# LulinZhang/BRDF-NeRF

Measured on AMD Instinct MI355X. Metric: train rays/sec (+ MFMA% of roofline), spsbrdf-nerf 64 samples/ray, 1/2/4/8 MI355X, higher is better.
Workload: dtype bf16; 1 GPU; BASELINE config 2: Djibouti-shaped synthetic rays, spsbrdf-nerf lambert train step (pass1 64 + guided 64 samples/ray, F=512, 8 Siren layers, PE10, ds_lambda=10), 4096 rays/GPU/step (4096 rays per global step, weak scaling); rays_per_gpu=4096, n_samples=64, guided_samples=64, parallelism=dp1, settle_steps=218

## Files before the change

brdf_nerf_amd/csrc/diag.h:

```cpp
#ifdef BN_SWITCH
BN_SWITCH(BN_PHASE_TIMING)
BN_SWITCH(BN_PHASE_TIMING_WGRAD)
BN_SWITCH(BN_CLOCK_STAMP)
BN_SWITCH(BN_CLOCK_STAMP_WGRAD)
BN_SWITCH(BN_TIMELINE)
BN_SWITCH(BN_GEMM_PRIO)
BN_SWITCH(BN_NO_NT_STASH)
BN_SWITCH(BN_NO_PINGPONG)
BN_SWITCH(BN_BWD_NO_PINGPONG)
BN_SWITCH(BN_FWD_DEPTH_TRAIN)
BN_SWITCH(BN_BWD_DEPTH)
BN_SWITCH(BN_BWD_PP_DEPTH)
BN_SWITCH(BN_BWD_D_AT)
BN_SWITCH(BN_NO_FLAT_COMPOSITE)
BN_SWITCH(SKINNY_SPLITS)
BN_SWITCH(BN_W2_BLOCKS)
BN_SWITCH(BN_DIAG_D8_IN_F32)
BN_SWITCH(BN_PROBE_NO_A)
BN_SWITCH(BN_PROBE_NO_B)
BN_SWITCH(BN_PROBE_NO_D)
BN_SWITCH(BN_PROBE_NO_RIDE)
BN_SWITCH(BN_ABLATION_BUILD)
#else
#ifndef BN_GEMM_PRIO
#define BN_GEMM_PRIO 1
#endif
#ifndef BN_FWD_DEPTH_TRAIN
#define BN_FWD_DEPTH_TRAIN 6
#endif
#ifndef BN_BWD_DEPTH
#define BN_BWD_DEPTH 2
#endif
#ifndef BN_BWD_PP_DEPTH
#define BN_BWD_PP_DEPTH 6
#endif
#ifndef BN_BWD_D_AT
#define BN_BWD_D_AT 0
#endif
#ifndef SKINNY_SPLITS
#define SKINNY_SPLITS 256
#endif
#ifndef BN_W2_BLOCKS
#define BN_W2_BLOCKS 256
#endif
#endif
```

brdf_nerf_amd/csrc/field_bwd.hip:

```cpp
#include "field_kernels.h"
#include "field_wgrad.h"

int bn_field_adjoint_backward(const bn_field_desc *desc, const bn_field_params *params, const void *packed, const bn_points *pts,
                              const float *d_out, void *stash, void *stream);

__device__ unsigned int g_bwd_fault;
unsigned int bn_bwd_fault_read(hipStream_t) {
  unsigned int v = 0u;
  if (hipMemcpyFromSymbol(&v, HIP_SYMBOL(g_bwd_fault), sizeof(unsigned int), 0, hipMemcpyDeviceToHost) != hipSuccess) return 0x80000000u;
  return v;
}
const unsigned int *bn_bwd_fault_ptr() {
  void *p = nullptr;
  return hipGetSymbolAddress(&p, HIP_SYMBOL(g_bwd_fault)) == hipSuccess ? (const unsigned int *)p : nullptr;
}

BN_PH_DEFINE_READER(bn_debug_phase_read_bwd)
BN_CLK_DEFINE(bn_debug_clock_read_bwd)

struct BwdArgs {
  FieldGeom g;
  bn_field_desc d;
  bn_field_params p;
  PackedLayout pl;
// ... 127 lines not shown
  const int N = g.pass_N[p];
  const int pc0 = wave * 32 * NTW;
  if (pc0 >= N) return;
  const int hl = pc0 / g.H2, hd = 2 * p + hl;
  const int nout = A.d.head_out[hd];
  const float *w2 = A.p.head_w2[hd];
  const char *DGs = A.stash + A.sl.DG[p] + (size_t)tile * dtile_bytes<DK>(BM, F);
#pragma unroll
  for (int nt = 0; nt < NTW; ++nt) {
    f32x4 wa[2][3], wb[2][3];
#pragma unroll
    for (int gp = 0; gp < 2; ++gp) {
      const int nl = pc0 + nt * 32 + 16 * gp + 4 * h - hl * g.H2;
#pragma unroll
      for (int c = 0; c < 3; ++c) {
        wa[gp][c] = c < nout ? *(const f32x4 *)(w2 + (size_t)c * g.H2 + nl) : f32x4{0, 0, 0, 0};
        wb[gp][c] = c < nout ? *(const f32x4 *)(w2 + (size_t)c * g.H2 + nl + 8) : f32x4{0, 0, 0, 0};
      }
    }
#pragma unroll
    for (int mt = 0; mt < MT; ++mt) {
      const int m = mt * 32 + r;
      const float d0 = DPH[m * BN_DPH + hd * 3 + 0], d1 = DPH[m * BN_DPH + hd * 3 + 1], d2 = DPH[m * BN_DPH + hd * 3 + 2];
      const DPiece<DK> pc = dpiece_load<DK>(DGs + dpiece_off<DK, MT, NTW>(wave, nt, mt, lane));
#pragma unroll
      for (int gp = 0; gp < 2; ++gp) {
        const int n0 = pc0 + nt * 32 + 16 * gp + 4 * h;
        float dg[8];
        dpiece_get<DK>(pc, gp, g.act, 1.f, dg);
        float va[4], vb[4];
#pragma unroll
        for (int e = 0; e < 4; ++e) {
          va[e] = (d0 * wa[gp][0][e] + d1 * wa[gp][1][e] + d2 * wa[gp][2][e]) * dg[e];
          vb[e] = (d0 * wb[gp][0][e] + d1 * wb[gp][1][e] + d2 * wb[gp][2][e]) * dg[4 + e];
        }
        *(vec4 *)(ACT + (size_t)m * LDA + n0) = to_vec4(T(), va[0], va[1], va[2], va[3]);
        *(vec4 *)(ACT + (size_t)m * LDA + n0 + 8) = to_vec4(T(), vb[0], vb[1], vb[2], vb[3]);
      }
    }
  }
}

template <typename T, int MT, int NT, int WAVES, bool D16>
__global__ __launch_bounds__(WAVES * 64, 2) void field_bwd_kernel(const BwdArgs A) {
  typedef typename DKind<T, D16>::type DK;
  typedef typename Elem<T>::vec4 vec4;
  constexpr int BM = MT * 32;
  extern __shared__ __attribute__((aligned(16))) char smem[];
  const FieldGeom &g = A.g;
  const int F = g.F, LDA = F + Elem<T>::kPad, KSF = F / 16;
  T *ACT = (T *)smem;
  float *DPH = (float *)(ACT + (size_t)BM * LDA);
  float *DPT = DPH + BM * BN_DPH;
  int *WR = (int *)(DPT + BM * 4), *RD = WR + 2;

  const int tid = threadIdx.x, lane = tid & 63, wave = tid >> 6, r = lane & 31, h = lane >> 5;
  const int64_t tile = blockIdx.x, m0 = tile * BM, M = A.M;
  const T *packed = (const T *)A.packed;
  constexpr int DP = (NT == 2 && WAVES == 8 && Elem<T>::kFastMath) ? (BN_BWD_PP_DEPTH | BN_GEMM_AFFINE) : BwdDepth<T>::value;
  constexpr int NPRE = std::is_same<DK, DK8>::value ? NT : 1;
  BN_PH_DECL
  BN_CLK_BEGIN

  const float gs = chain_scale(A.amax);
  if (tid < 16) WR[tid] = 0;
  if (tid < BM) {
    const int m = tid;
    const int64_t gm = m0 + m;
    float dph[BN_DPH], dpt[4];
    bwd_dpre(A, gm, dph, dpt);
    float *sh = (float *)(A.stash + A.sl.dpre_head) + gm * BN_DPH;
    float *st = (float *)(A.stash + A.sl.dpre_trunk) + gm * 4;
#pragma unroll
    for (int i = 0; i < BN_DPH; ++i) { DPH[m * BN_DPH + i] = dph[i] * gs; sh[i] = dph[i]; }
#pragma unroll
    for (int i = 0; i < 4; ++i) { DPT[m * 4 + i] = dpt[i] * gs; st[i] = dpt[i]; }
  }
  __syncthreads();
  BN_PH(0)

  const int ncol0 = wave * 32 * NT;
  const bool wave_on = ncol0 < F;
  const int n_on = F / (32 * NT) < WAVES ? F / (32 * NT) : WAVES;
  const bool ride = NT == 2 ? true : tile_copy_exact(F, n_on, WAVES);
  f32x16 acc[NT][MT];
  zero_acc<MT, NT>(acc);
  const float zr = (A.an && A.amax) ? gs / grad_scale_from(A.amax + 1, BN_GS_TARGET_ADJ) : 1.f;

  for (int p = 0; p < g.n_pass; ++p) {
    if (g.pass_heads[p] == 2) bwd_head_dG<T, MT, NT, D16>(A, p, ACT, DPH, m0, tile);
    else bwd_head_dG<T, MT, BN_SINGLE_HEAD_NTW(NT), D16>(A, p, ACT, DPH, m0, tile);
    BN_PH(1)
    __syncthreads();
    BN_PH(2)
    BN_PH(3)
    const int KSp = g.pass_N[p] / 16;
    tile_to_global<T>(ACT, LDA, (T *)(A.stash + A.sl.dG[p]) + (size_t)m0 * g.pass_N[p], g.pass_N[p], BM, g.pass_N[p]);
    if (wave_on) gemm_seg<T, MT, NT, DP>(acc, packed + A.pl.bwd_head[p] + (size_t)(ncol0 / 32) * KSp * 512, KSp, ACT, LDA, lane);
    BN_PH(4)
    __syncthreads();
    BN_PH(5)
  }
  if (wave_on && !g.fold) {
#pragma unroll
    for (int nt = 0; nt < NT; ++nt)
#pragma unroll
      for (int gq = 0; gq < 4; ++gq) {
        const int n = ncol0 + nt * 32 + 8 * gq + 4 * h;
#pragma unroll
        for (int mt = 0; mt < MT; ++mt) {
          const int m = mt * 32 + r;
          *(vec4 *)(ACT + (size_t)m * LDA + n) =
              to_vec4(T(), acc[nt][mt][4 * gq], acc[nt][mt][4 * gq + 1], acc[nt][mt][4 * gq + 2], acc[nt][mt][4 * gq + 3]);
        }
      }
  }
  BN_PH(6)
  __syncthreads();
// ... 83 lines not shown
            }
#pragma unroll
            for (int e = 0; e < 8; ++e) v[e] += zb[e] * zr;
          }
          if constexpr (NATZ) {
            const typename Elem<T>::frag q = cvt8(T(), v);
            *(vec4 *)(ACT + (size_t)m * LDA + n0) = __builtin_shufflevector(q, q, 0, 1, 2, 3);
            *(vec4 *)(ACT + (size_t)m * LDA + n0 + 8) = __builtin_shufflevector(q, q, 4, 5, 6, 7);
            stash_store_buf(Zr, voff, ((((wave_u * NT + nt) * MT + mt) * 2 + gp) * 1024), q);
          } else {
            *(vec4 *)(ACT + (size_t)m * LDA + n0) = to_vec4(T(), v[0], v[1], v[2], v[3]);
            *(vec4 *)(ACT + (size_t)m * LDA + n0 + 8) = to_vec4(T(), v[4], v[5], v[6], v[7]);
          }
        }
      }
  };
  {
    if (!g.fold) {
      zero_acc<MT, NT>(acc);
      T *fdst = (T *)(A.stash + A.sl.dfeats) + (size_t)m0 * F;
      if (!ride) tile_to_global<T>(ACT, LDA, fdst, F, BM, F);
      if (wave_on) {
        load_D(g.L - 1, 0, NPRE);
        const size_t off = A.pl.bwd_feats + (size_t)(ncol0 / 32) * KSF * 512;
        if (ride) {
          TileCopyExact<T> zcopy(ACT, LDA, fdst, F, F, tid, WAVES * 64);
          gemm_seg<T, MT, NT, DP>(acc, packed + off, KSF, ACT, LDA, lane, zcopy);
        } else {
          gemm_seg<T, MT, NT, DP>(acc, packed + off, KSF, ACT, LDA, lane);
        }
        load_D(g.L - 1, NPRE, NT);
      }
    } else if (wave_on) {
      load_D(g.L - 1, 0, NT);
    }
    BN_PH(9)
    __syncthreads();
    BN_PH(10)
    if (wave_on) epilogue(g.L - 1, std::true_type());
    BN_PH(11)
    __syncthreads();
    BN_PH(12)
  }
  for (int l = g.L - 1; l >= 1; --l) {
    const int it = g.L - 1 - l;
    const int lo = l - 1;
    zero_acc<MT, NT>(acc);
    T *zdst = (T *)(A.stash + A.sl.dZ[l]) + (size_t)m0 * F;
    if (!NATZ && !ride) tile_to_global<T>(ACT, LDA, zdst, F, BM, F);
    if (wave_on) {
      if (!PING || BN_BWD_D_AT == 0) load_D(lo, 0, NPRE);
      const size_t off = A.pl.bwd_trunk[l] + (size_t)(ncol0 / 32) * KSF * 512;
      if constexpr (PING) {
        pp_wait(WR + 0, 4 * it, &g_bwd_fault);
        if (grp == 1) pp_wait(RD + 0, 4 * (it + 1), &g_bwd_fault);
        BN_PH(12)
        __builtin_amdgcn_s_setprio(1);
        if constexpr (sizeof(T) == 2) {
          gemm_fixed<T, MT, NT, (DP & (BN_GEMM_AFFINE - 1)), 32, 16>(acc, packed + off, KSF, 0, ACT, LDA, lane, [&]() {
            pp_signal(RD + 0 + grp, lane);
            pp_wait(WR + 1, 4 * it, &g_bwd_fault);
            if (BN_BWD_D_AT == 1) load_D(lo, 0, NPRE);
          });
        }
        __builtin_amdgcn_s_setprio(0);
        pp_signal(RD + 2 + grp, lane);
        if (BN_BWD_D_AT == 2) load_D(lo, 0, NPRE);
      } else if (!NATZ && ride) {
        TileCopyExact<T> zcopy(ACT, LDA, zdst, F, F, tid, WAVES * 64);
        gemm_seg<T, MT, NT, DP>(acc, packed + off, KSF, ACT, LDA, lane, zcopy);
      } else {
        gemm_seg<T, MT, NT, DP>(acc, packed + off, KSF, ACT, LDA, lane);
      }
      load_D(lo, NPRE, NT);
    }
    BN_PH(9)
    if constexpr (PING) {
      pp_wait(RD + 2 * grp + 0, 4 * (it + 1), &g_bwd_fault);
      pp_wait(RD + 2 * grp + 1, 4 * (it + 1), &g_bwd_fault);
    } else {
      __syncthreads();
    }
    BN_PH(10)
    if (wave_on) epilogue(lo, std::false_type());
    BN_PH(11)
    if constexpr (PING) pp_signal(WR + grp, lane);
    else __syncthreads();
    BN_PH(12)
  }
  if (PING) __syncthreads();
  if (!NATZ) tile_to_global<T>(ACT, LDA, (T *)(A.stash + A.sl.dZ[0]) + (size_t)m0 * F, F, BM, F);
  BN_PH(13)
#ifndef BN_PHASE_TIMING_WGRAD
  BN_PH_FLUSH
#endif
#ifndef BN_CLOCK_STAMP_WGRAD
  BN_CLK_END
#endif
}

template <typename T, int MT, int NT, int WAVES, bool D16> static int launch_bwd_k(const BwdArgs &a, int64_t tiles, hipStream_t st) {
  constexpr int BM = MT * 32;
  const size_t lds = (size_t)BM * (a.g.F + Elem<T>::kPad) * sizeof(T) + (size_t)BM * (BN_DPH + 4) * sizeof(float) + 64;
  if (int e = bn_configure_lds((const void *)field_bwd_kernel<T, MT, NT, WAVES, D16>, lds, "field_bwd")) return e;
  BnProfScope prof_(BN_K_BWD_CHAIN, st);
  field_bwd_kernel<T, MT, NT, WAVES, D16><<<dim3((unsigned)tiles), WAVES * 64, lds, st>>>(a);
  BN_LAUNCH_CHECK("field_bwd");
  return 0;
}
template <typename T, int MT, int NT, int WAVES> static int launch_bwd(const BwdArgs &a, int64_t tiles, hipStream_t st) {
  if constexpr (std::is_same<T, f16>::value) {
    if (a.g.dsz == 2) return launch_bwd_k<T, MT, NT, WAVES, true>(a, tiles, st);
  }
  return launch_bwd_k<T, MT, NT, WAVES, false>(a, tiles, st);
}

extern "C" int bn_field_backward(const bn_field_desc *desc, const bn_field_params *params, const void *packed,
                                 const bn_points *pts, const float *out, const float *d_out, void *stash,
                                 const bn_field_grads *G, void *stream) {
  return bn_field_backward_parts(desc, params, packed, pts, out, d_out, stash, G, BN_BWD_ALL, stream);
}

extern "C" int bn_field_backward_parts(const bn_field_desc *desc, const bn_field_params *params, const void *packed,
                                       const bn_points *pts, const float *out, const float *d_out, void *stash,
                                       const bn_field_grads *G, int32_t parts, void *stream) {
  BwdArgs a;
  if (int e = bn_make_geom(desc, &a.g)) return e;
  if (const int f = bn_field_fault_seen()) {
    bn_set_error("field_backward: an earlier %s launch lost an LDS hand-over (pp_wait timed out): its results are invalid",
                 (f & 1) ? "forward" : "backward");
    return BN_ELAUNCH;
  }
  a.an = desc->normal_an ? 1 : 0;
  BN_REQUIRE(pts && pts->n_points > 0 && packed && out && d_out && stash && G, "field_backward: null argument");
  BN_REQUIRE(parts > 0 && (parts & ~BN_BWD_ALL) == 0, "field_backward: parts=%d", parts);
  BN_REQUIRE(pts->point_offset == 0 && (pts->total_points == 0 || pts->total_points == pts->n_points),
             "field_backward: the backward runs over a whole point set (point_offset = 0)");
  BN_REQUIRE(pts->seg1_points == 0 || (pts->rays && pts->z && pts->z2 && pts->n_samples2 > 0 && pts->seg1_points < pts->n_points &&
                                       pts->seg1_points % pts->n_samples == 0 && (pts->n_points - pts->seg1_points) % pts->n_samples2 == 0),
// ... 165 lines not shown
```

brdf_nerf_amd/csrc/field_fwd.hip:

```cpp
#include "field_kernels.h"

struct FwdArgs {
  FieldGeom g;
  bn_field_desc d;
  bn_field_params p;
  PackedLayout pl;
  StashLayout sl;
  const void *packed;
  bn_points pts;
  float *out;
  char *stash;
  int sigma_only;
};

#define BN_INV_2PI 0.15915494309189535f

__device__ unsigned int g_fwd_fault;
static unsigned int *g_fault_host = nullptr;
static unsigned int g_fwd_launches = 0;
const unsigned int *bn_fwd_fault_ptr() {
  void *p = nullptr;
  return hipGetSymbolAddress(&p, HIP_SYMBOL(g_fwd_fault)) == hipSuccess ? (const unsigned int *)p : nullptr;
}

// ... 190 lines not shown
  constexpr int BM = MT * 32;
  constexpr int PADE = Elem<T>::kPad;
  constexpr bool FAST = Elem<T>::kFastMath;
  constexpr bool NATY = Elem<T>::kNativeY;
  constexpr int DP = FwdDepth<T, KEEP>::value;
  extern __shared__ __attribute__((aligned(16))) char smem[];
  const FieldGeom &g = A.g;
  const int F = g.F, LDA = F + PADE, KP = g.KP, LDP = KP + PADE;
  T *ACT = (T *)smem;
  T *PE = ACT + (size_t)BM * LDA;
  float *RED = (float *)(PE + (size_t)BM * LDP);

  const int tid = threadIdx.x, lane = tid & 63, wave = tid >> 6;
  const int r = lane & 31, h = lane >> 5;
  const int64_t tile = blockIdx.x, m0 = tile * BM, M = A.pts.n_points;
  const T *packed = (const T *)A.packed;
  constexpr bool keep = KEEP;
  BN_PH_DECL
  BN_CLK_BEGIN

  {
    constexpr int NP = (WAVES * 64) / BM;
    const int m = tid % BM, part = tid / BM;
    const int64_t gm = m0 + m;
    float x[3] = {0.f, 0.f, 0.f};
    if (gm < M) {
      if (A.pts.xyz) {
        x[0] = A.pts.xyz[gm * 3 + 0]; x[1] = A.pts.xyz[gm * 3 + 1]; x[2] = A.pts.xyz[gm * 3 + 2];
      } else {
        const int64_t ray = gm / A.pts.n_samples;
        const float *rr = A.pts.rays + ray * A.pts.ray_stride;
        const float zz = A.pts.z[gm];
        x[0] = rr[0] + rr[3] * zz; x[1] = rr[1] + rr[4] * zz; x[2] = rr[2] + rr[5] * zz;
      }
    }
    T *row = PE + (size_t)m * LDP;
    if (g.pe_freqs > 0) {
      for (int k = part; k < g.pe_freqs; k += NP) {
        const float f = (float)(1 << k);
#pragma unroll
        for (int c = 0; c < 3; ++c) {
          float s, co;
          sincos_t<FAST>(f * x[c], s, co);
          row[6 * k + c] = (T)s;
          row[6 * k + 3 + c] = (T)co;
        }
      }
      if (part == 0)
        for (int k = g.P; k < KP; ++k) row[k] = (T)0.f;
    } else if (part == 0) {
      for (int k = 0; k < KP; ++k) row[k] = (T)(k < 3 ? x[k] : 0.f);
    }
  }
  if (tid < 8) ((int *)RED)[tid] = 0;
  __syncthreads();
  if (keep) tile_to_global<T>(PE, LDP, (T *)(A.stash + A.sl.pe) + (size_t)m0 * KP, KP, BM, KP);
  BN_PH(0)

  const int ncol0 = wave * 32 * NT;
  const bool wave_on = ncol0 < F;
  const int KSP = KP / 16, KSF = F / 16;
  f32x16 acc[NT][MT];

  const int n_on = F / (32 * NT) < WAVES ? F / (32 * NT) : WAVES;
  const bool ride = NT == 2 ? true : tile_copy_exact(F, n_on, WAVES);
#ifndef BN_NO_PINGPONG
  constexpr bool PING = NT == 2 && WAVES == 8 && FAST;
#else
  constexpr bool PING = false;
#endif
  int *WR = (int *)RED, *RD = WR + 2;
  const int grp = wave >> 2;
  BN_TL_DECL((char *)RED + 64 + 4096)
  float *BIASL = (float *)((char *)RED + 64) + wave * 128;
  float bnext = 0.f;
  const int wave_u = __builtin_amdgcn_readfirstlane(wave);
  if constexpr (PING) BIASL[lane] = A.p.trunk_b[0][ncol0 + lane] * act_prescale<FAST>(g.act, 30.f);
  for (int l = 0; l < g.L; ++l) {
    BN_TL(0)
    if constexpr (PING) {
      if (l + 1 < g.L) bnext = A.p.trunk_b[l + 1][ncol0 + lane];
      const float *bl = BIASL + (l & 1) * 64 + 4 * h;
#pragma unroll
      for (int nt = 0; nt < NT; ++nt)
#pragma unroll
        for (int gp = 0; gp < 2; ++gp) {
          const f32x4 b0 = *(const f32x4 *)(bl + nt * 32 + 16 * gp), b1 = *(const f32x4 *)(bl + nt * 32 + 16 * gp + 8);
#pragma unroll
          for (int mt = 0; mt < MT; ++mt)
#pragma unroll
            for (int e = 0; e < 4; ++e) { acc[nt][mt][8 * gp + e] = b0[e]; acc[nt][mt][8 * gp + 4 + e] = b1[e]; }
        }
    } else {
      zero_acc<MT, NT>(acc);
    }
    if (keep && !NATY && !ride && l > 0) tile_to_global<T>(ACT, LDA, (T *)(A.stash + A.sl.Y[l - 1]) + (size_t)m0 * F, F, BM, F);
    if (wave_on) {
      const size_t t0 = (size_t)(ncol0 / 32);
      const T *w_pe = packed + A.pl.fwd_trunk[l][0] + t0 * KSP * 512;
      const T *w_h = packed + A.pl.fwd_trunk[l][l == g.skip ? 1 : 0] + t0 * KSF * 512;
      if (l == 0 || l == g.skip) gemm_seg<T, MT, NT, DP>(acc, w_pe, KSP, PE, LDP, lane);
      if (l > 0) {
        if (PING) {
          BN_PH(1)
          pp_wait(WR + 0, 4 * l, &g_fwd_fault);
          if (grp == 1) pp_wait(RD + 0, 4 * l, &g_fwd_fault);
          BN_PH(12)
          BN_TL(1)
          __builtin_amdgcn_s_setprio(BN_GEMM_PRIO);
          if constexpr (sizeof(T) == 2) {
            gemm_fixed<T, MT, NT, (DP & (BN_GEMM_AFFINE - 1)), 32, 16>(acc, w_h, KSF, 0, ACT, LDA, lane, [&]() {
              BN_TL(2)
              pp_signal(RD + 0 + grp, lane);
              pp_wait(WR + 1, 4 * l, &g_fwd_fault);
              BN_TL(3)
            });
          }
          __builtin_amdgcn_s_setprio(0);
          BN_TL(4)
          pp_signal(RD + 2 + grp, lane);
        } else if (keep && !NATY && ride) {
          TileCopyExact<T> ycopy(ACT, LDA, (T *)(A.stash + A.sl.Y[l - 1]) + (size_t)m0 * F, F, F, tid, WAVES * 64);
          gemm_seg<T, MT, NT, DP>(acc, w_h, KSF, ACT, LDA, lane, ycopy);
        } else {
          gemm_seg<T, MT, NT, DP>(acc, w_h, KSF, ACT, LDA, lane);
        }
      }
    }
    const float w0 = (l == 0) ? 30.f : 1.f;
    f32x4 bia[NT][2][2];
    if constexpr (PING) {
      if (l + 1 < g.L) BIASL[((l + 1) & 1) * 64 + lane] = bnext * act_prescale<FAST>(g.act, 1.f);
    } else if (wave_on) {
      const float bscale = act_prescale<FAST>(g.act, w0);
      const float *bias = A.p.trunk_b[l];
#pragma unroll
      for (int nt = 0; nt < NT; ++nt)
#pragma unroll
        for (int gp = 0; gp < 2; ++gp) {
          const int n0 = ncol0 + nt * 32 + 16 * gp + 4 * h;
          bia[nt][gp][0] = *(const f32x4 *)(bias + n0) * bscale;
          bia[nt][gp][1] = *(const f32x4 *)(bias + n0 + 8) * bscale;
        }
    }
    BN_PH(1)
    if constexpr (PING) {
      const auto Yr = stash_rsrc(keep ? A.stash + A.sl.Y[l] + (size_t)tile * BM * F * sizeof(T) : nullptr);
      const auto Dr = stash_rsrc(keep ? A.stash + A.sl.D[l] + (size_t)tile * dtile_bytes<DK>(BM, F) : nullptr);
      const int voff = lane * 16;
      auto passes = [&](auto act_tag) {
        typedef typename Elem<T>::frag frag;
        constexpr int ACTK = decltype(act_tag)::value;
        const float dsc = ACTK == BN_ACT_SIN ? w0 : 1.f;
        if (l > 0) {
          pp_wait(RD + 2 * grp + 0, 4 * l, &g_fwd_fault);
          pp_wait(RD + 2 * grp + 1, 4 * l, &g_fwd_fault);
        }
        BN_PH(2)
        BN_TL(5)
#pragma unroll
        for (int nt = 0; nt < NT; ++nt) {
          DHalf<DK> dh0[MT];
#pragma unroll
          for (int gp = 0; gp < 2; ++gp) {
            const int n0 = ncol0 + nt * 32 + 16 * gp + 4 * h;
#pragma unroll
            for (int mt = 0; mt < MT; ++mt) {
              float y[8], c[8];
#pragma unroll
              for (int e = 0; e < 8; ++e) act_eval<FAST, ACTK>(acc[nt][mt][8 * gp + e], w0, y[e], c[e]);
              const int m = mt * 32 + r;
              const frag yq = cvt8(T(), y);
              *(vec4 *)(ACT + (size_t)m * LDA + n0) = __builtin_shufflevector(yq, yq, 0, 1, 2, 3);
              *(vec4 *)(ACT + (size_t)m * LDA + n0 + 8) = __builtin_shufflevector(yq, yq, 4, 5, 6, 7);
              if (keep) {
                stash_store_buf(Yr, voff, ((((wave_u * NT + nt) * MT + mt) * 2 + gp) * 1024), yq);
                if (gp == 0) dh0[mt] = dhalf_make<DK>(c, dsc);
                else dpiece_store_buf<DK>(Dr, voff, (wave_u * NT + nt) * MT + mt, dh0[mt], dhalf_make<DK>(c, dsc));
              }
            }
          }
        }
        BN_TL(6)
        pp_signal(WR + grp, lane);
        BN_PH(3)
      };
      if (g.act == BN_ACT_SIN) passes(std::integral_constant<int, BN_ACT_SIN>());
      else passes(std::integral_constant<int, BN_ACT_RELU>());
      BN_PH(4)
    } else {
    __syncthreads();
    BN_PH(2)
    if (wave_on) {
      char *Ds = keep ? A.stash + A.sl.D[l] + (size_t)tile * dtile_bytes<DK>(BM, F) : nullptr;
      T *Ys = keep ? (T *)(A.stash + A.sl.Y[l]) + (size_t)tile * BM * F : nullptr;
      auto epilogue = [&](auto act_tag) {
        constexpr int ACTK = decltype(act_tag)::value;
        const float dsc = ACTK == BN_ACT_SIN ? w0 : 1.f;
#pragma unroll
        for (int nt = 0; nt < NT; ++nt) {
          DHalf<DK> dh0[MT];
#pragma unroll
          for (int gp = 0; gp < 2; ++gp) {
            const int n0 = ncol0 + nt * 32 + 16 * gp + 4 * h;
            const f32x4 ba = bia[nt][gp][0], bb = bia[nt][gp][1];
#pragma unroll
            for (int mt = 0; mt < MT; ++mt) {
              float y[8], dd[8];
#pragma unroll
              for (int e = 0; e < 4; ++e) {
                act_eval<FAST, ACTK>(acc[nt][mt][8 * gp + e] + ba[e], w0, y[e], dd[e]);
                act_eval<FAST, ACTK>(acc[nt][mt][8 * gp + 4 + e] + bb[e], w0, y[4 + e], dd[4 + e]);
              }
              const int m = mt * 32 + r;
              if (NATY) {
                const typename Elem<T>::frag yq = cvt8(T(), y);
                *(vec4 *)(ACT + (size_t)m * LDA + n0) = __builtin_shufflevector(yq, yq, 0, 1, 2, 3);
                *(vec4 *)(ACT + (size_t)m * LDA + n0 + 8) = __builtin_shufflevector(yq, yq, 4, 5, 6, 7);
                if (keep) st_frag(Ys + native_off8<MT, NT>(wave, nt, mt, gp, lane), yq);
              } else {
                *(vec4 *)(ACT + (size_t)m * LDA + n0) = to_vec4(T(), y[0], y[1], y[2], y[3]);
                *(vec4 *)(ACT + (size_t)m * LDA + n0 + 8) = to_vec4(T(), y[4], y[5], y[6], y[7]);
              }
              if (keep) {
                if (gp == 0) dh0[mt] = dhalf_make<DK>(dd, dsc);
                else dpiece_store<DK>(Ds + dpiece_off<DK, MT, NT>(wave, nt, mt, lane), dh0[mt], dhalf_make<DK>(dd, dsc));
              }
            }
          }
        }
      };
      if (g.act == BN_ACT_SIN) epilogue(std::integral_constant<int, BN_ACT_SIN>());
      else epilogue(std::integral_constant<int, BN_ACT_RELU>());
    }
    BN_PH(3)
    __syncthreads();
    BN_PH(4)
// ... 403 lines not shown
```

brdf_nerf_amd/csrc/field_kernels.h:

```cpp
#pragma once
#include "field.h"
#include "instrument.h"

typedef __attribute__((ext_vector_type(4))) unsigned int u32x4;
typedef __attribute__((ext_vector_type(2))) unsigned int u32x2;
template <typename V> __device__ __forceinline__ void stash_store(V *p, const V &v) {
#ifdef BN_NO_NT_STASH
  *p = v;
#else
  __builtin_nontemporal_store(v, p);
#endif
}
template <typename V> __device__ __forceinline__ V stash_load(const V *p) {
#ifdef BN_NO_NT_STASH
  return *p;
#else
  return __builtin_nontemporal_load(p);
#endif
}

__device__ __forceinline__ auto stash_rsrc(const void *base) {
  const unsigned long long b = (unsigned long long)base;
  const unsigned int lo = __builtin_amdgcn_readfirstlane((unsigned int)b), hi = __builtin_amdgcn_readfirstlane((unsigned int)(b >> 32));
  return __builtin_amdgcn_make_buffer_rsrc((void *)(((unsigned long long)hi << 32) | lo), 0, 0x7fffffff, 0x00020000);
// ... 20 lines not shown
    }                                                                                            \
    if ((G).NT == 2) return FN<float, 2, 2, 8> ARGS;                                             \
    return FN<float, 2, 1, 8> ARGS;                                                              \
  } while (0)


template <typename T> __device__ __forceinline__ typename Elem<T>::frag lds_frag(const T *p);
template <> __device__ __forceinline__ bf16x8 lds_frag<bf16>(const bf16 *p) { return *(const bf16x8 *)p; }
template <> __device__ __forceinline__ f16x8 lds_frag<f16>(const f16 *p) { return *(const f16x8 *)p; }
template <> __device__ __forceinline__ f32x8 lds_frag<float>(const float *p) {
  f32x4 a = *(const f32x4 *)p, b = *(const f32x4 *)(p + 4);
  f32x8 r = {a[0], a[1], a[2], a[3], b[0], b[1], b[2], b[3]};
  return r;
}

struct NoSide {
  __device__ __forceinline__ void at(int) const {}
};

template <typename T> struct TileCopyExact {
  static constexpr int EPC = 16 / sizeof(T);
  const T *lp;
  T *gp;
  int lstep, gstep;
  __device__ __forceinline__ TileCopyExact(const T *lds, int ld, T *g, int gld, int width, int t, int nthr) {
    const int cpr = width / EPC, row = t / cpr, cc = t % cpr, dr = nthr / cpr;
    lp = lds + (size_t)row * ld + cc * EPC;
    gp = g + (size_t)row * gld + cc * EPC;
    lstep = dr * ld; gstep = dr * gld;
  }
  __device__ __forceinline__ void at(int parity) {
    if (parity == 0) {
#ifndef BN_PROBE_NO_RIDE
      stash_store((u32x4 *)gp, *(const u32x4 *)lp);
#endif
      lp += lstep; gp += gstep;
    }
  }
};
__host__ __device__ __forceinline__ bool tile_copy_exact(int F, int n_on, int waves) { return n_on == waves && F % 256 == 0; }

typedef __attribute__((address_space(3))) int lds_int;
__device__ __forceinline__ void pp_wait(int *flag, int target, unsigned int *fault) {
  volatile lds_int *f = (volatile lds_int *)flag;
  int spin = 0;
  for (; *f < target && spin < (1 << 24); ++spin) __builtin_amdgcn_s_sleep(1);
  if (spin >= (1 << 24) && (threadIdx.x & 63) == 0) atomicOr(fault, 1u);
  asm volatile("" ::: "memory");
}
__device__ __forceinline__ void pp_signal(int *flag, int lane) {
  asm volatile("s_waitcnt lgkmcnt(0)" ::: "memory");
  if (lane == 0) __hip_atomic_fetch_add((lds_int *)flag, 1, __ATOMIC_RELAXED, __HIP_MEMORY_SCOPE_WORKGROUP);
}

#define BN_GEMM_AFFINE 64
template <typename T, bool TRAIN_FWD> struct FwdDepth { static constexpr int value = 4; };
template <> struct FwdDepth<bf16, true> { static constexpr int value = BN_FWD_DEPTH_TRAIN | BN_GEMM_AFFINE; };
template <> struct FwdDepth<f16, true> { static constexpr int value = BN_FWD_DEPTH_TRAIN | BN_GEMM_AFFINE; };
template <typename T> struct BwdDepth { static constexpr int value = Elem<T>::kFastMath ? BN_BWD_DEPTH : 4; };

template <typename T, int MT, int NTW, int DEPTH_, typename Side>
__device__ __forceinline__ void gemm_range(f32x16 (&acc)[NTW][MT], const T *__restrict__ wp, int KS, int ks0, int nks, const T *bsrc,
                                           int ldb, int lane, Side &side) {
  constexpr int DEPTH = DEPTH_ & (BN_GEMM_AFFINE - 1);
  constexpr bool AFFINE = (DEPTH_ & BN_GEMM_AFFINE) != 0;
  typedef typename Elem<T>::frag frag;
  static_assert(DEPTH % 2 == 0, "side jobs rely on an even pipeline depth");
  const int r = lane & 31, h = lane >> 5;
  const T *wl = wp + (size_t)lane * 8;
  const T *bl = bsrc + (size_t)r * ldb + 8 * h;
  const int kend = ks0 + nks;
  frag A[DEPTH][NTW];
  auto loadA = [&](frag(&a)[NTW], int ks) {
    ks = ks < kend ? ks : kend - 1;
    {
#pragma unroll
      for (int nt = 0; nt < NTW; ++nt) {
#ifdef BN_PROBE_NO_A
        if (ks >= ks0 + DEPTH) { asm volatile("" : "+v"(a[nt])); continue; }
#endif
        a[nt] = lds_frag<T>(wl + ((size_t)nt * KS + ks) * 512);
      }
    }
  };
  auto loadB = [&](frag(&B)[MT], int ks) {
#pragma unroll
    for (int mt = 0; mt < MT; ++mt) {
#ifdef BN_PROBE_NO_B
      if (ks != ks0) { asm volatile("" : "+v"(B[mt])); continue; }
#endif
      B[mt] = lds_frag<T>(bl + (size_t)mt * 32 * ldb + ks * 16);
    }
  };
  frag Bc[MT];
  auto step = [&](frag(&a)[NTW], int ks) {
    frag Bn[MT];
    loadB(Bn, ks + 1 < kend ? ks + 1 : ks0);
#pragma unroll
    for (int nt = 0; nt < NTW; ++nt)
#pragma unroll
      for (int mt = 0; mt < MT; ++mt) mma32(acc[nt][mt], a[nt], Bc[mt]);
#pragma unroll
    for (int mt = 0; mt < MT; ++mt) Bc[mt] = Bn[mt];
  };
#pragma unroll
  for (int d = 0; d < DEPTH; ++d) loadA(A[d], ks0 + d);
  loadB(Bc, ks0);
  __builtin_amdgcn_sched_barrier(0);
  int ks = ks0;
  if constexpr (AFFINE) {
  {
    const T *bm[MT];
#pragma unroll
    for (int mt = 0; mt < MT; ++mt) bm[mt] = bl + (size_t)mt * 32 * ldb + (size_t)ks0 * 16;
    for (; ks + DEPTH <= kend; ks += DEPTH) {
#pragma unroll
      for (int d = 0; d < DEPTH; ++d) {
        frag Bn[MT];
#pragma unroll
        for (int mt = 0; mt < MT; ++mt) Bn[mt] = lds_frag<T>(bm[mt] + (d + 1) * 16);
#pragma unroll
        for (int nt = 0; nt < NTW; ++nt)
#pragma unroll
          for (int mt = 0; mt < MT; ++mt) mma32(acc[nt][mt], A[d][nt], Bc[mt]);
#pragma unroll
        for (int mt = 0; mt < MT; ++mt) Bc[mt] = Bn[mt];
        loadA(A[d], ks + d + DEPTH);
        side.at(d & 1);
        __builtin_amdgcn_sched_barrier(0);
      }
#pragma unroll
      for (int mt = 0; mt < MT; ++mt) bm[mt] += DEPTH * 16;
    }
  }
  } else {
  for (; ks + DEPTH <= kend; ks += DEPTH) {
#pragma unroll
    for (int d = 0; d < DEPTH; ++d) {
      step(A[d], ks + d);
      loadA(A[d], ks + d + DEPTH);
      side.at(d & 1);
      __builtin_amdgcn_sched_barrier(0);
    }
  }
  }
#pragma unroll
  for (int d = 0; d < DEPTH; ++d)
    if (ks + d < kend) {
      step(A[d], ks + d);
      side.at(d & 1);
    }
}
struct NoMid {
  __device__ __forceinline__ void operator()() const {}
};
template <typename T, int MT, int NTW, int DEPTH, int NKS, int MID, typename Mid, typename Side = NoSide>
__device__ __forceinline__ void gemm_fixed(f32x16 (&acc)[NTW][MT], const T *__restrict__ wp, int KS, int ks0, const T *bsrc, int ldb,
                                           int lane, Mid &&mid, Side &&side = Side()) {
  typedef typename Elem<T>::frag frag;
  static_assert(sizeof(frag) == 16, "16-bit modes only: one 16-byte fragment piece per lane");
  static_assert(MID >= 0 && MID < NKS && DEPTH <= NKS && (MID == 0 || DEPTH <= MID), "the ring must not wrap inside the prologue");
  const int r = lane & 31, h = lane >> 5;
  const T *bm[MT];
#pragma unroll
  for (int mt = 0; mt < MT; ++mt) bm[mt] = bsrc + (size_t)(r + 32 * mt) * ldb + 8 * h + (size_t)ks0 * 16;
  const auto rs = stash_rsrc(wp);
  const int voff = lane * 16;
  auto ldA = [&](int nt, int ks) {
    return __builtin_bit_cast(frag, __builtin_amdgcn_raw_buffer_load_b128(rs, voff, (nt * KS + ks0 + ks) * (512 * (int)sizeof(T)), 0));
  };
  frag A[DEPTH][NTW], Bc[MT];
#pragma unroll
  for (int d = 0; d < DEPTH; ++d)
#pragma unroll
    for (int nt = 0; nt < NTW; ++nt) A[d][nt] = ldA(nt, d);
#pragma unroll
  for (int mt = 0; mt < MT; ++mt) Bc[mt] = lds_frag<T>(bm[mt]);
  __builtin_amdgcn_sched_barrier(0);
#pragma unroll
  for (int j = 0; j < NKS; ++j) {
    const bool ahead = j + 1 < NKS && (MID == 0 || j + 1 != MID);
    frag Bn[MT];
    if (ahead) {
#pragma unroll
      for (int mt = 0; mt < MT; ++mt) Bn[mt] = lds_frag<T>(bm[mt] + (j + 1) * 16);
    }
#pragma unroll
    for (int nt = 0; nt < NTW; ++nt)
#pragma unroll
      for (int mt = 0; mt < MT; ++mt) mma32(acc[nt][mt], A[j % DEPTH][nt], Bc[mt]);
    if (ahead) {
#pragma unroll
      for (int mt = 0; mt < MT; ++mt) Bc[mt] = Bn[mt];
    }
    if (j + DEPTH < NKS) {
#pragma unroll
      for (int nt = 0; nt < NTW; ++nt) A[j % DEPTH][nt] = ldA(nt, j + DEPTH);
    }
    side.at(j & 1);
    __builtin_amdgcn_sched_barrier(0);
    if (MID > 0 && j + 1 == MID) {
      mid();
#pragma unroll
      for (int mt = 0; mt < MT; ++mt) Bc[mt] = lds_frag<T>(bm[mt] + MID * 16);
      __builtin_amdgcn_sched_barrier(0);
    }
  }
}
template <typename T, int MT, int NTW, int DEPTH, typename Side>
__device__ __forceinline__ void gemm_seg(f32x16 (&acc)[NTW][MT], const T *__restrict__ wp, int KS, const T *bsrc, int ldb,
                                         int lane, Side &side) {
  gemm_range<T, MT, NTW, DEPTH>(acc, wp, KS, 0, KS, bsrc, ldb, lane, side);
}
template <typename T, int MT, int NTW, int DEPTH>
__device__ __forceinline__ void gemm_seg(f32x16 (&acc)[NTW][MT], const T *__restrict__ wp, int KS, const T *bsrc, int ldb,
                                         int lane) {
  NoSide none;
  gemm_range<T, MT, NTW, DEPTH>(acc, wp, KS, 0, KS, bsrc, ldb, lane, none);
}

template <typename T, int MT, int NTW, int DP, bool HOT, typename Side = NoSide>
__device__ __forceinline__ void gemm_full(f32x16 (&acc)[NTW][MT], const T *__restrict__ wp, int KS, const T *bsrc, int ldb, int lane,
                                          Side &&side = Side()) {
  if constexpr (HOT && sizeof(T) == 2) {
    constexpr int D = (DP & (BN_GEMM_AFFINE - 1)) < 2 ? 2 : (DP & (BN_GEMM_AFFINE - 1));
    if (KS == 32) { gemm_fixed<T, MT, NTW, D, 32, 0>(acc, wp, KS, 0, bsrc, ldb, lane, NoMid(), side); return; }
    if constexpr (std::is_same<std::decay_t<Side>, NoSide>::value) {
      if (KS == 16) { gemm_fixed<T, MT, NTW, D, 16, 0>(acc, wp, KS, 0, bsrc, ldb, lane, NoMid()); return; }
    }
  }
  gemm_seg<T, MT, NTW, DP>(acc, wp, KS, bsrc, ldb, lane, side);
}

template <int MT, int NTW> __device__ __forceinline__ void zero_acc(f32x16 (&acc)[NTW][MT]) {
#pragma unroll
  for (int nt = 0; nt < NTW; ++nt)
#pragma unroll
    for (int mt = 0; mt < MT; ++mt)
#pragma unroll
      for (int i = 0; i < 16; ++i) acc[nt][mt][i] = 0.f;
}

template <int MT, int NTW> __device__ __forceinline__ size_t native_off8(int wave, int nt, int mt, int gp, int lane) {
  return ((((size_t)(wave * NTW + nt) * MT + mt) * 2 + gp) * 64 + lane) * 8;
}
__device__ __forceinline__ bf16x8 cvt8(bf16, const float (&v)[8]) {
  bf16x8 o;
#pragma unroll
  for (int i = 0; i < 8; ++i) o[i] = (bf16)v[i];
  return o;
}
__device__ __forceinline__ f16x8 cvt8(f16, const float (&v)[8]) {
  const f32x8 f = {v[0], v[1], v[2], v[3], v[4], v[5], v[6], v[7]};
  return __builtin_convertvector(f, f16x8);
}
__device__ __forceinline__ f32x8 cvt8(float, const float (&v)[8]) {
  const f32x8 f = {v[0], v[1], v[2], v[3], v[4], v[5], v[6], v[7]};
// ... 137 lines not shown
```

profiles/simd_timeline.py:

```python
import ctypes
import os
import subprocess
import sys

ROOT = os.path.dirname(os.path.dirname(os.path.abspath(__file__)))
sys.path.insert(0, ROOT)
from brdf_nerf_amd import build as B

EV = {0: "layer", 1: "g0+", 2: "g0-", 3: "g1+", 4: "g1-", 5: "S+", 6: "S-", 7: "C+", 8: "C-", 9: "end", 10: "Sc-"}
NEV, NBLK = 112, 8


def build_tl(defines, tag):
    B.build()
    objdir = os.path.join(B.HERE, "build")
    objs = [os.path.join(objdir, os.path.basename(s) + ".o") for s in B.sources() if not s.endswith("field_fwd.hip")]
    obj = os.path.join(objdir, f"field_fwd.hip.timeline{tag}.o")
    subprocess.check_call(B.compile_command(os.path.join(B.CSRC, "field_fwd.hip"), obj, ["BN_TIMELINE"] + list(defines)))
    lib = os.path.join(objdir, f"libbn_timeline{tag}.so")
    subprocess.check_call([B.HIPCC, "--offload-arch=gfx950", "-shared", "-fPIC", "-o", lib] + objs + [obj])
    return lib


def intervals(events, a, b):
    out, t0 = [], None
    for code, t in events:
        if code == a:
            t0 = t
        elif code == b and t0 is not None:
            out.append((t0, t))
            t0 = None
    return out


def covered(ivs, lo, hi, step=64):
    n = (hi - lo) // step + 1
    m = [0] * n
    for t0, t1 in ivs:
        for i in range(max(0, (t0 - lo) // step), min(n, (t1 - lo) // step + 1)):
            m[i] = 1
    return m


if __name__ == "__main__":
    defines = [a[2:] for a in sys.argv[1:] if a.startswith("-D")]
    tag = "".join("_" + d.replace("=", "") for d in defines)
    lib = os.path.join(B.HERE, "build", f"libbn_timeline{tag}.so") if "--no-build" in sys.argv else build_tl(defines, tag)
    if "--build-only" in sys.argv:
        sys.exit(0)
    nblk = int(sys.argv[sys.argv.index("--blocks") + 1]) if "--blocks" in sys.argv else 2
    from brdf_nerf_amd import _lib
    _lib.LIB_PATH = lib
    import torch
    import bench
    from brdf_nerf_amd import load_model
    from brdf_nerf_amd import functions as Fn
    L = _lib.lib()
    L.bn_debug_timeline_read_fwd.argtypes = [ctypes.c_void_p]
    dev = torch.device("cuda", 0)
    args = bench.make_args(4096, 64, 64, "bf16")
    torch.manual_seed(0)
    model = load_model(args).to(dev)
    spec = model.spec(False, False, False)
    packed = model.repack(spec)
    b = bench.synthetic_batch(4096, 1, dev)
    z = torch.sort(torch.rand(4096, 64, device=dev) * 2, -1)[0]
    n = z.numel()
    out = torch.empty(n, spec.out_channels, device=dev)
    stash = torch.empty(Fn.field_stash_bytes(spec, n), dtype=torch.uint8, device=dev)
    sigma = "--sigma" in sys.argv
    run = (lambda: Fn.field_sigma(spec, model.named(), packed, rays=b["rays"], z=z)) if sigma else \
        (lambda: Fn.field_forward_raw(spec, model.named(), packed, out, stash, rays=b["rays"], z=z))
    for _ in range(20):
        run()
    torch.cuda.synchronize()
    buf = (ctypes.c_ulonglong * (NBLK * 8 * NEV))()
    assert L.bn_debug_timeline_read_fwd(buf) == 0
    print("variant:", defines or "default", "| kernel:", "sigma-only inference forward" if sigma else "training forward (stash)",
          "| 262,144 points, bf16, F = 512; cycles = s_memtime ticks from the workgroup's first stamp")
    print("events: g0 / g1 = GEMM over input-column half 0 / 1, S = pass S (sin, pack, LDS tile + Y stash; 'Sc' = its arithmetic done,",
          "group 0 then waits for the readers), C = pass C (cos, 8-bit D stash)")
    tot = {"one": 0, "both": 0, "none": 0}
    for blk in range(nblk):
        waves = []
        for w in range(8):
            raw = [buf[(blk * 8 + w) * NEV + i] for i in range(NEV)]
            hw = raw[0]
            ev = [(int(x >> 56), int(x & ((1 << 56) - 1))) for x in raw[1:] if x]
            waves.append((hw, ev))
        t0 = min(ev[0][1] for hw, ev in waves if ev)
        print(f"\nworkgroup {blk}")
        for simd_pair in range(4):
            wa, wb = simd_pair, simd_pair + 4
            print(f"  waves {wa} (group 0) and {wb} (group 1): HW_ID simd {(waves[wa][0] >> 4) & 3} / {(waves[wb][0] >> 4) & 3}, cu {(waves[wa][0] >> 8) & 15} / {(waves[wb][0] >> 8) & 15}")
            for w in (wa, wb):
                hw, ev = waves[w]
                line, layer = [], -1
                for code, t in ev:
                    if code == 0:
                        layer += 1
                        line.append(f"\n      L{layer}:")
                    else:
                        line.append(f"{EV.get(code, code)}{t - t0}")
                print(f"    wave {w}:" + " ".join(line))
            if blk == 0 or True:
                ga = intervals(waves[wa][1], 1, 2) + intervals(waves[wa][1], 3, 4)
                gb = intervals(waves[wb][1], 1, 2) + intervals(waves[wb][1], 3, 4)
                if ga and gb:
                    lo = min(ga[0][0], gb[0][0])
                    hi = max(e[1] for e in waves[wa][1] + waves[wb][1] if e[0] == 9)
                    ma, mb = covered(ga, lo, hi), covered(gb, lo, hi)
                    one = sum(1 for x, y in zip(ma, mb) if x + y == 1)
                    both = sum(1 for x, y in zip(ma, mb) if x + y == 2)
                    none = len(ma) - one - both
                    tot["one"] += one; tot["both"] += both; tot["none"] += none
                    print(f"    layers 1-7 ({hi - lo} cycles): one wave in a GEMM {100 * one / len(ma):.1f} %, both {100 * both / len(ma):.1f} %, neither {100 * none / len(ma):.1f} %")
    s = sum(tot.values())
    if s:
        print(f"\nall SIMD pairs of {nblk} workgroups: one wave in a GEMM {100 * tot['one'] / s:.1f} %, both {100 * tot['both'] / s:.1f} %, neither {100 * tot['none'] / s:.1f} %")
```

Baseline: 613,000 rays/s.

## Split ping-pong GEMM hand-over into four K-quarters with lagged counters

The producer/consumer ping-pong between the two wave groups in the forward and backward field kernels previously handed over at one midpoint, splitting K into halves. It now hands over at every quarter of K (HO=8 of 16 k-steps per segment granularity), using per-quarter LDS counters. A configurable lag (BN_FWD_LAG/BN_BWD_LAG) sets how many quarters group 1 trails group 0. The aim is finer-grained overlap of one group's GEMM with the other group's activation passes, shrinking idle gaps on shared SIMDs. The cost is more LDS atomic signal/wait points, plus extra ring refills at each hand-over that may stall the MFMA pipeline.

```diff
diff --git a/brdf_nerf_amd/csrc/diag.h b/brdf_nerf_amd/csrc/diag.h
--- a/brdf_nerf_amd/csrc/diag.h
+++ b/brdf_nerf_amd/csrc/diag.h
@@ -5,6 +5,8 @@
 BN_SWITCH(BN_CLOCK_STAMP_WGRAD)
 BN_SWITCH(BN_TIMELINE)
 BN_SWITCH(BN_GEMM_PRIO)
+BN_SWITCH(BN_FWD_LAG)
+BN_SWITCH(BN_BWD_LAG)
 BN_SWITCH(BN_NO_NT_STASH)
 BN_SWITCH(BN_NO_PINGPONG)
 BN_SWITCH(BN_BWD_NO_PINGPONG)
@@ -25,6 +27,12 @@
 #ifndef BN_GEMM_PRIO
 #define BN_GEMM_PRIO 1
 #endif
+#ifndef BN_FWD_LAG
+#define BN_FWD_LAG 2
+#endif
+#ifndef BN_BWD_LAG
+#define BN_BWD_LAG 2
+#endif
 #ifndef BN_FWD_DEPTH_TRAIN
 #define BN_FWD_DEPTH_TRAIN 6
 #endif
diff --git a/brdf_nerf_amd/csrc/field_bwd.hip b/brdf_nerf_amd/csrc/field_bwd.hip
--- a/brdf_nerf_amd/csrc/field_bwd.hip
+++ b/brdf_nerf_amd/csrc/field_bwd.hip
@@ -203,7 +203,7 @@
   T *ACT = (T *)smem;
   float *DPH = (float *)(ACT + (size_t)BM * LDA);
   float *DPT = DPH + BM * BN_DPH;
-  int *WR = (int *)(DPT + BM * 4), *RD = WR + 2;
+  int *CT = (int *)(DPT + BM * 4);
 
   const int tid = threadIdx.x, lane = tid & 63, wave = tid >> 6, r = lane & 31, h = lane >> 5;
   const int64_t tile = blockIdx.x, m0 = tile * BM, M = A.M;
@@ -214,7 +214,7 @@
   BN_CLK_BEGIN
 
   const float gs = chain_scale(A.amax);
-  if (tid < 16) WR[tid] = 0;
+  if (tid < 16) CT[tid] = 0;
   if (tid < BM) {
     const int m = tid;
     const int64_t gm = m0 + m;
@@ -404,19 +404,19 @@
       if (!PING || BN_BWD_D_AT == 0) load_D(lo, 0, NPRE);
       const size_t off = A.pl.bwd_trunk[l] + (size_t)(ncol0 / 32) * KSF * 512;
       if constexpr (PING) {
-        pp_wait(WR + 0, 4 * it, &g_bwd_fault);
-        if (grp == 1) pp_wait(RD + 0, 4 * (it + 1), &g_bwd_fault);
+        pp_wait(pp_wr(CT, 0), 2 * it, &g_bwd_fault);
+        if (grp == 1) pp_wait(pp_rd(CT, BN_BWD_LAG - 1, 0), 4 * (it + 1), &g_bwd_fault);
         BN_PH(12)
         __builtin_amdgcn_s_setprio(1);
         if constexpr (sizeof(T) == 2) {
-          gemm_fixed<T, MT, NT, (DP & (BN_GEMM_AFFINE - 1)), 32, 16>(acc, packed + off, KSF, 0, ACT, LDA, lane, [&]() {
-            pp_signal(RD + 0 + grp, lane);
-            pp_wait(WR + 1, 4 * it, &g_bwd_fault);
-            if (BN_BWD_D_AT == 1) load_D(lo, 0, NPRE);
+          gemm_fixed<T, MT, NT, (DP & (BN_GEMM_AFFINE - 1)), 32, 8>(acc, packed + off, KSF, 0, ACT, LDA, lane, [&](int q) {
+            pp_signal(pp_rd(CT, q - 1, grp), lane);
+            pp_wait(pp_wr(CT, q), 2 * it, &g_bwd_fault);
+            if (BN_BWD_D_AT == 1 && q == 2) load_D(lo, 0, NPRE);
           });
         }
         __builtin_amdgcn_s_setprio(0);
-        pp_signal(RD + 2 + grp, lane);
+        pp_signal(pp_rd(CT, 3, grp), lane);
         if (BN_BWD_D_AT == 2) load_D(lo, 0, NPRE);
       } else if (!NATZ && ride) {
         TileCopyExact<T> zcopy(ACT, LDA, zdst, F, F, tid, WAVES * 64);
@@ -428,15 +428,15 @@
     }
     BN_PH(9)
     if constexpr (PING) {
-      pp_wait(RD + 2 * grp + 0, 4 * (it + 1), &g_bwd_fault);
-      pp_wait(RD + 2 * grp + 1, 4 * (it + 1), &g_bwd_fault);
+      pp_wait(pp_rd(CT, wave_u >> 1, 0), 4 * (it + 1), &g_bwd_fault);
+      pp_wait(pp_rd(CT, wave_u >> 1, 1), 4 * (it + 1), &g_bwd_fault);
     } else {
       __syncthreads();
     }
     BN_PH(10)
     if (wave_on) epilogue(lo, std::false_type());
     BN_PH(11)
-    if constexpr (PING) pp_signal(WR + grp, lane);
+    if constexpr (PING) pp_signal(pp_wr(CT, wave_u >> 1), lane);
     else __syncthreads();
     BN_PH(12)
   }
diff --git a/brdf_nerf_amd/csrc/field_fwd.hip b/brdf_nerf_amd/csrc/field_fwd.hip
--- a/brdf_nerf_amd/csrc/field_fwd.hip
+++ b/brdf_nerf_amd/csrc/field_fwd.hip
@@ -266,7 +266,7 @@
       for (int k = 0; k < KP; ++k) row[k] = (T)(k < 3 ? x[k] : 0.f);
     }
   }
-  if (tid < 8) ((int *)RED)[tid] = 0;
+  if (tid < 16) ((int *)RED)[tid] = 0;
   __syncthreads();
   if (keep) tile_to_global<T>(PE, LDP, (T *)(A.stash + A.sl.pe) + (size_t)m0 * KP, KP, BM, KP);
   BN_PH(0)
@@ -283,7 +283,7 @@
 #else
   constexpr bool PING = false;
 #endif
-  int *WR = (int *)RED, *RD = WR + 2;
+  int *CT = (int *)RED;
   const int grp = wave >> 2;
   BN_TL_DECL((char *)RED + 64 + 4096)
   float *BIASL = (float *)((char *)RED + 64) + wave * 128;
@@ -317,22 +317,22 @@
       if (l > 0) {
         if (PING) {
           BN_PH(1)
-          pp_wait(WR + 0, 4 * l, &g_fwd_fault);
-          if (grp == 1) pp_wait(RD + 0, 4 * l, &g_fwd_fault);
+          pp_wait(pp_wr(CT, 0), 2 * l, &g_fwd_fault);
+          if (grp == 1) pp_wait(pp_rd(CT, BN_FWD_LAG - 1, 0), 4 * l, &g_fwd_fault);
           BN_PH(12)
           BN_TL(1)
           __builtin_amdgcn_s_setprio(BN_GEMM_PRIO);
           if constexpr (sizeof(T) == 2) {
-            gemm_fixed<T, MT, NT, (DP & (BN_GEMM_AFFINE - 1)), 32, 16>(acc, w_h, KSF, 0, ACT, LDA, lane, [&]() {
+            gemm_fixed<T, MT, NT, (DP & (BN_GEMM_AFFINE - 1)), 32, 8>(acc, w_h, KSF, 0, ACT, LDA, lane, [&](int q) {
               BN_TL(2)
-              pp_signal(RD + 0 + grp, lane);
-              pp_wait(WR + 1, 4 * l, &g_fwd_fault);
+              pp_signal(pp_rd(CT, q - 1, grp), lane);
+              pp_wait(pp_wr(CT, q), 2 * l, &g_fwd_fault);
               BN_TL(3)
             });
           }
           __builtin_amdgcn_s_setprio(0);
           BN_TL(4)
-          pp_signal(RD + 2 + grp, lane);
+          pp_signal(pp_rd(CT, 3, grp), lane);
         } else if (keep && !NATY && ride) {
           TileCopyExact<T> ycopy(ACT, LDA, (T *)(A.stash + A.sl.Y[l - 1]) + (size_t)m0 * F, F, F, tid, WAVES * 64);
           gemm_seg<T, MT, NT, DP>(acc, w_h, KSF, ACT, LDA, lane, ycopy);
@@ -367,8 +367,8 @@
         constexpr int ACTK = decltype(act_tag)::value;
         const float dsc = ACTK == BN_ACT_SIN ? w0 : 1.f;
         if (l > 0) {
-          pp_wait(RD + 2 * grp + 0, 4 * l, &g_fwd_fault);
-          pp_wait(RD + 2 * grp + 1, 4 * l, &g_fwd_fault);
+          pp_wait(pp_rd(CT, wave_u >> 1, 0), 4 * l, &g_fwd_fault);
+          pp_wait(pp_rd(CT, wave_u >> 1, 1), 4 * l, &g_fwd_fault);
         }
         BN_PH(2)
         BN_TL(5)
@@ -396,7 +396,7 @@
           }
         }
         BN_TL(6)
-        pp_signal(WR + grp, lane);
+        pp_signal(pp_wr(CT, wave_u >> 1), lane);
         BN_PH(3)
       };
       if (g.act == BN_ACT_SIN) passes(std::integral_constant<int, BN_ACT_SIN>());
diff --git a/brdf_nerf_amd/csrc/field_kernels.h b/brdf_nerf_amd/csrc/field_kernels.h
--- a/brdf_nerf_amd/csrc/field_kernels.h
+++ b/brdf_nerf_amd/csrc/field_kernels.h
@@ -96,6 +96,9 @@
   asm volatile("s_waitcnt lgkmcnt(0)" ::: "memory");
   if (lane == 0) __hip_atomic_fetch_add((lds_int *)flag, 1, __ATOMIC_RELAXED, __HIP_MEMORY_SCOPE_WORKGROUP);
 }
+
+__device__ __forceinline__ int *pp_rd(int *ct, int q, int g) { return ct + 4 * q + g; }
+__device__ __forceinline__ int *pp_wr(int *ct, int q) { return ct + 4 * q + 2; }
 
 #define BN_GEMM_AFFINE 64
 template <typename T, bool TRAIN_FWD> struct FwdDepth { static constexpr int value = 4; };
@@ -196,14 +199,14 @@
     }
 }
 struct NoMid {
-  __device__ __forceinline__ void operator()() const {}
+  __device__ __forceinline__ void operator()(int) const {}
 };
-template <typename T, int MT, int NTW, int DEPTH, int NKS, int MID, typename Mid, typename Side = NoSide>
+template <typename T, int MT, int NTW, int DEPTH, int NKS, int HO, typename Mid, typename Side = NoSide>
 __device__ __forceinline__ void gemm_fixed(f32x16 (&acc)[NTW][MT], const T *__restrict__ wp, int KS, int ks0, const T *bsrc, int ldb,
                                            int lane, Mid &&mid, Side &&side = Side()) {
   typedef typename Elem<T>::frag frag;
   static_assert(sizeof(frag) == 16, "16-bit modes only: one 16-byte fragment piece per lane");
-  static_assert(MID >= 0 && MID < NKS && DEPTH <= NKS && (MID == 0 || DEPTH <= MID), "the ring must not wrap inside the prologue");
+  static_assert(HO >= 0 && HO < NKS && DEPTH <= NKS && (HO == 0 || (DEPTH <= HO && NKS % HO == 0)), "the ring must not wrap inside the prologue");
   const int r = lane & 31, h = lane >> 5;
   const T *bm[MT];
 #pragma unroll
@@ -223,7 +226,8 @@
   __builtin_amdgcn_sched_barrier(0);
 #pragma unroll
   for (int j = 0; j < NKS; ++j) {
-    const bool ahead = j + 1 < NKS && (MID == 0 || j + 1 != MID);
+    const bool handover = HO > 0 && j + 1 < NKS && (j + 1) % (HO > 0 ? HO : 1) == 0;
+    const bool ahead = j + 1 < NKS && !handover;
     frag Bn[MT];
     if (ahead) {
 #pragma unroll
@@ -243,10 +247,10 @@
     }
     side.at(j & 1);
     __builtin_amdgcn_sched_barrier(0);
-    if (MID > 0 && j + 1 == MID) {
-      mid();
-#pragma unroll
-      for (int mt = 0; mt < MT; ++mt) Bc[mt] = lds_frag<T>(bm[mt] + MID * 16);
+    if (handover) {
+      mid((j + 1) / (HO > 0 ? HO : 1));
+#pragma unroll
+      for (int mt = 0; mt < MT; ++mt) Bc[mt] = lds_frag<T>(bm[mt] + (j + 1) * 16);
       __builtin_amdgcn_sched_barrier(0);
     }
   }
diff --git a/profiles/simd_timeline.py b/profiles/simd_timeline.py
--- a/profiles/simd_timeline.py
+++ b/profiles/simd_timeline.py
@@ -7,7 +7,7 @@
 sys.path.insert(0, ROOT)
 from brdf_nerf_amd import build as B
 
-EV = {0: "layer", 1: "g0+", 2: "g0-", 3: "g1+", 4: "g1-", 5: "S+", 6: "S-", 7: "C+", 8: "C-", 9: "end", 10: "Sc-"}
+EV = {0: "layer", 1: "q+", 2: "q-", 3: "q+", 4: "q-", 5: "S+", 6: "S-", 7: "C+", 8: "C-", 9: "end", 10: "Sc-"}
 NEV, NBLK = 112, 8
 
 
@@ -23,11 +23,12 @@
 
 
 def intervals(events, a, b):
+    a, b = (a if isinstance(a, tuple) else (a,)), (b if isinstance(b, tuple) else (b,))
     out, t0 = [], None
     for code, t in events:
-        if code == a:
+        if code in a:
             t0 = t
-        elif code == b and t0 is not None:
+        elif code in b and t0 is not None:
             out.append((t0, t))
             t0 = None
     return out
@@ -78,7 +79,7 @@
     assert L.bn_debug_timeline_read_fwd(buf) == 0
     print("variant:", defines or "default", "| kernel:", "sigma-only inference forward" if sigma else "training forward (stash)",
           "| 262,144 points, bf16, F = 512; cycles = s_memtime ticks from the workgroup's first stamp")
-    print("events: g0 / g1 = GEMM over input-column half 0 / 1, S = pass S (sin, pack, LDS tile + Y stash; 'Sc' = its arithmetic done,",
+    print("events: q+ / q- = start / end of the GEMM over one input-column quarter (four per layer: the gap between a q- and the next q+ is the hand-over wait), S = pass S (sin, pack, LDS tile + Y stash; 'Sc' = its arithmetic done,",
           "group 0 then waits for the readers), C = pass C (cos, 8-bit D stash)")
     tot = {"one": 0, "both": 0, "none": 0}
     for blk in range(nblk):
@@ -104,8 +105,8 @@
                         line.append(f"{EV.get(code, code)}{t - t0}")
                 print(f"    wave {w}:" + " ".join(line))
             if blk == 0 or True:
-                ga = intervals(waves[wa][1], 1, 2) + intervals(waves[wa][1], 3, 4)
-                gb = intervals(waves[wb][1], 1, 2) + intervals(waves[wb][1], 3, 4)
+                ga = intervals(waves[wa][1], (1, 3), (2, 4))
+                gb = intervals(waves[wb][1], (1, 3), (2, 4))
                 if ga and gb:
                     lo = min(ga[0][0], gb[0][0])
                     hi = max(e[1] for e in waves[wa][1] + waves[wb][1] if e[0] == 9)
```

Result: no change. 610,600 rays/s, median of 2 (-0.4%).
